# nju-websoft/OpenEA

Hardware: AMD Instinct MI355X
Metric: training triples/sec (k=10 truncated negatives + limited loss + Adagrad) (higher is better)
Workload: dtype f32; 1 GPU; BootEA/AlignE translational step, EN-FR-100K-V1 shape (synthetic), dim=100, GLOBAL batch=20000 positives (weak scaling: 20000 per GPU x 1 GPU), k=10, truncated eps=0.98; the same workload at every N (; global_batch=20000, entities=200000, parallelism=single

## Files before the change

### openea_amd/csrc/triple_step.hip

```cpp
#include <stdlib.h>

#include <algorithm>
#include <vector>

#include "common.h"
#include "step_plan.h"

namespace {

using oea::group_sum;

using oea::flag_t;
using oea::grad_t;

struct StepWs {
    grad_t *ent_grad, *rel_grad;
    grad_t *rel_extra;
    int64_t rel_copy_stride;
    flag_t *ent_touched, *rel_touched;
    grad_t *nrm_grad, *nrm_extra;
    flag_t *nrm_touched;
    double *partials;
    __device__ __forceinline__ grad_t *rel_copy(int64_t c) const {
        return c == 0 ? rel_grad : rel_extra + (c - 1) * rel_copy_stride;
    }
    __device__ __forceinline__ grad_t *nrm_copy(int64_t c) const {
        return c == 0 ? nrm_grad : nrm_extra + (c - 1) * rel_copy_stride;
    }
};
constexpr int kMaxBlocks = 4096;
constexpr int kRelCopies = 16;

static size_t align256(size_t x) { return (x + 255) / 256 * 256; }

static size_t ws_layout(int64_t n_ent, int64_t n_rel, int32_t ld, void *base, StepWs *ws) {
    size_t off = 0;
    char *b = static_cast<char *>(base);
    auto take = [&](size_t bytes) { size_t o = off; off += align256(bytes); return b ? b + o : nullptr; };
    grad_t *eg = (grad_t *)take(sizeof(grad_t) * (size_t)n_ent * ld);
    grad_t *rg = (grad_t *)take(sizeof(grad_t) * (size_t)n_rel * ld);
    grad_t *ng = (grad_t *)take(sizeof(grad_t) * (size_t)n_rel * ld);
    flag_t *et = (flag_t *)take(sizeof(flag_t) * (size_t)n_ent);
    flag_t *rt = (flag_t *)take(sizeof(flag_t) * (size_t)n_rel);
    flag_t *nt = (flag_t *)take(sizeof(flag_t) * (size_t)n_rel);
    grad_t *rx = (grad_t *)take(sizeof(grad_t) * (size_t)n_rel * ld * (kRelCopies - 1));
    grad_t *nx = (grad_t *)take(sizeof(grad_t) * (size_t)n_rel * ld * (kRelCopies - 1));
    double *pp = (double *)take(sizeof(double) * kMaxBlocks);
    if (ws) {
        ws->rel_copy_stride = n_rel * (int64_t)ld; ws->ent_grad = eg; ws->rel_grad = rg; ws->rel_extra = rx;
        ws->ent_touched = et; ws->rel_touched = rt; ws->nrm_grad = ng; ws->nrm_extra = nx; ws->nrm_touched = nt; ws->partials = pp;
    }
    return off;
}

template <int G, int IT>
struct Row {
    float v[IT];
};

template <int G, int IT, bool TIGHT = false>
__device__ __forceinline__ void load_row(const float *__restrict__ base, int ld, int lane, Row<G, IT> &r) {
#pragma unroll
    for (int it = 0; it < IT; ++it) {
        const int c = it * G + lane;
        r.v[it] = ((TIGHT && G == 32 && it < IT - 1) || c < ld) ? base[c] : 0.f;
    }
}
template <int G, int IT>
__device__ __forceinline__ void load_grad_raw(const grad_t *__restrict__ base, int ld, int lane, grad_t (&q)[IT]) {
#pragma unroll
    for (int it = 0; it < IT; ++it) {
        const int c = it * G + lane;
        q[it] = c < ld ? base[c] : (grad_t)0;
    }
}
template <int G, int IT>
__device__ __forceinline__ void load_grad_row(const grad_t *__restrict__ base, int ld, int lane, Row<G, IT> &r) {
#pragma unroll
    for (int it = 0; it < IT; ++it) {
        const int c = it * G + lane;
        r.v[it] = c < ld ? oea::grad_val(base[c]) : 0.f;
    }
}
template <int G, int IT>
__device__ __forceinline__ float sumsq(const Row<G, IT> &r) {
    float s = 0.f;
#pragma unroll
    for (int it = 0; it < IT; ++it) s += r.v[it] * r.v[it];
    return group_sum<G>(s);
}
template <int G, int IT>
__device__ __forceinline__ void normalize(Row<G, IT> &r, int on) {
    if (!on) return;
    const float inv = rsqrtf(fmaxf(sumsq<G, IT>(r), 1e-12f));
#pragma unroll
    for (int it = 0; it < IT; ++it) r.v[it] *= inv;
}
template <int G, int IT>
__device__ __forceinline__ float score(const Row<G, IT> &yh, const Row<G, IT> &yr, const Row<G, IT> &yt, int l1,
                                       Row<G, IT> &delta) {
    float s = 0.f;
#pragma unroll
    for (int it = 0; it < IT; ++it) {
        const float d = yh.v[it] + yr.v[it] - yt.v[it];
        delta.v[it] = d;
        s += l1 ? fabsf(d) : d * d;
    }
    return group_sum<G>(s);
}
__device__ __forceinline__ float sgn(float x) { return x > 0.f ? 1.f : (x < 0.f ? -1.f : 0.f); }

template <int G, int IT>
__device__ __forceinline__ void dscore(const Row<G, IT> &delta, float coef, int l1, Row<G, IT> &g) {
#pragma unroll
    for (int it = 0; it < IT; ++it) g.v[it] = l1 ? coef * sgn(delta.v[it]) : 2.f * coef * delta.v[it];
}
template <int G, int IT, bool SKIPZERO = true>
__device__ __forceinline__ void atomic_row(grad_t *__restrict__ dst, int ld, int lane, const Row<G, IT> &g, float sign) {
#pragma unroll
    for (int it = 0; it < IT; ++it) {
        const int c = it * G + lane;
        const float v = sign * g.v[it];
        if (((G == 32 && it < IT - 1) || c < ld) && (!SKIPZERO || v != 0.f)) oea::grad_add(dst + c, v);
    }
}

__device__ __forceinline__ float softplusf_(float x) { return x > 0.f ? x + log1pf(expf(-x)) : log1pf(expf(x)); }
__device__ __forceinline__ float sigmoidf_(float x) { return 1.f / (1.f + expf(-x)); }

__device__ __forceinline__ void triple_coef_kind(int loss_kind, const oea_step_cfg &cfg, bool is_pos, float s, float &coef,
                                                 float &l) {
    coef = 0.f; l = 0.f;
    switch (loss_kind) {
    case OEA_LOSS_LIMITED:
        if (is_pos) { const float x = s - cfg.pos_margin; if (x > 0.f) { l = x; coef = 1.f; } }
        else { const float x = cfg.neg_margin - s; if (x > 0.f) { l = cfg.balance * x; coef = -cfg.balance; } }
        break;
    case OEA_LOSS_LOGISTIC:
        if (is_pos) { l = softplusf_(s); coef = sigmoidf_(s); }
        else { l = softplusf_(-s); coef = -sigmoidf_(-s); }
        break;
    case OEA_LOSS_POSITIVE:
        l = s; coef = 1.f;
        break;
    case OEA_LOSS_ALIGN:
        l = softplusf_(s); coef = sigmoidf_(s);
        break;
    default: break;
    }
}
__device__ __forceinline__ void triple_coef(const oea_step_cfg &cfg, bool is_pos, float s, float &coef, float &l) {
    triple_coef_kind(cfg.loss_kind, cfg, is_pos, s, coef, l);
}

__device__ __forceinline__ void block_loss_partial(double loss_local, double *partials) {
    __shared__ double sred[4];
    const double w = oea::wave_sum_d(loss_local);
    if ((threadIdx.x & 63) == 0) sred[threadIdx.x >> 6] = w;
    __syncthreads();
    if (threadIdx.x == 0) partials[blockIdx.x] = sred[0] + sred[1] + sred[2] + sred[3];
}

template <int G, int IT>
__global__ __launch_bounds__(256) void triple_generic(
    const float *__restrict__ ent, const float *__restrict__ rel, int ld, const int32_t *__restrict__ pos,
    int64_t n_pos, const int32_t *__restrict__ neg, int64_t n_neg, oea_step_cfg cfg, StepWs ws) {
    const int lane = threadIdx.x % G;
    const int64_t grp = ((int64_t)blockIdx.x * blockDim.x + threadIdx.x) / G;
    const int64_t ngrp = (int64_t)gridDim.x * blockDim.x / G;
    const bool margin = cfg.loss_kind == OEA_LOSS_MARGIN;
    const int64_t items = margin ? n_pos : n_pos + n_neg;
    double loss_local = 0.0;
    for (int64_t item = grp; item < items; item += ngrp) {
        const bool is_pos = margin || item < n_pos;
        const int32_t *tr = is_pos ? pos + 3 * item : neg + 3 * (item - n_pos);
        const int h = tr[0], r = tr[1], t = tr[2];
        Row<G, IT> yh, yr, yt, delta, g;
        load_row<G, IT>(ent + (int64_t)h * ld, ld, lane, yh);
        load_row<G, IT>(rel + (int64_t)r * ld, ld, lane, yr);
        load_row<G, IT>(ent + (int64_t)t * ld, ld, lane, yt);
        normalize<G, IT>(yh, cfg.ent_l2_norm);
        normalize<G, IT>(yr, cfg.rel_l2_norm);
        normalize<G, IT>(yt, cfg.ent_l2_norm);
        const float s = score<G, IT>(yh, yr, yt, cfg.l1, delta);
        float coef, l;
        if (margin) {
            const int32_t *tn = neg + 3 * item;
            const int nh = tn[0], nr = tn[1], nt = tn[2];
            Row<G, IT> zh, zr, zt, dn;
            load_row<G, IT>(ent + (int64_t)nh * ld, ld, lane, zh);
            load_row<G, IT>(rel + (int64_t)nr * ld, ld, lane, zr);
            load_row<G, IT>(ent + (int64_t)nt * ld, ld, lane, zt);
            normalize<G, IT>(zh, cfg.ent_l2_norm);
            normalize<G, IT>(zr, cfg.rel_l2_norm);
            normalize<G, IT>(zt, cfg.ent_l2_norm);
            const float sn = score<G, IT>(zh, zr, zt, cfg.l1, dn);
            const float x = cfg.margin + s - sn;
            if (x <= 0.f) continue;
            if (lane == 0) loss_local += (double)x;
            dscore<G, IT>(dn, -1.f, cfg.l1, g);
            atomic_row<G, IT>(ws.ent_grad + (int64_t)nh * ld, ld, lane, g, 1.f);
            atomic_row<G, IT>(ws.rel_copy(item % kRelCopies) + (int64_t)nr * ld, ld, lane, g, 1.f);
            atomic_row<G, IT>(ws.ent_grad + (int64_t)nt * ld, ld, lane, g, -1.f);
            if (lane == 0) { ws.ent_touched[nh] = 1.f; ws.ent_touched[nt] = 1.f; ws.rel_touched[nr] = 1.f; }
            coef = 1.f;
        } else {
            triple_coef(cfg, is_pos, s, coef, l);
            if (lane == 0) loss_local += (double)l;
            if (coef == 0.f) continue;
        }
        dscore<G, IT>(delta, coef, cfg.l1, g);
        atomic_row<G, IT>(ws.ent_grad + (int64_t)h * ld, ld, lane, g, 1.f);
        atomic_row<G, IT>(ws.rel_copy(item % kRelCopies) + (int64_t)r * ld, ld, lane, g, 1.f);
        atomic_row<G, IT>(ws.ent_grad + (int64_t)t * ld, ld, lane, g, -1.f);
        if (lane == 0) { ws.ent_touched[h] = 1.f; ws.ent_touched[t] = 1.f; ws.rel_touched[r] = 1.f; }
    }
    block_loss_partial(loss_local, ws.partials);
}

template <int G, int IT>
__device__ __forceinline__ double score_independent(const float *__restrict__ ent, const float *__restrict__ rel, int ld,
                                                    int lane, int64_t item, int ch, int cr, int ct, bool is_pos,
                                                    const oea_step_cfg &cfg, const StepWs &ws, int lk, int l1) {
    Row<G, IT> zh, zr, zt, delta, g;
    load_row<G, IT>(ent + (int64_t)ch * ld, ld, lane, zh);
    load_row<G, IT>(rel + (int64_t)cr * ld, ld, lane, zr);
    load_row<G, IT>(ent + (int64_t)ct * ld, ld, lane, zt);
    normalize<G, IT>(zh, cfg.ent_l2_norm);
    normalize<G, IT>(zr, cfg.rel_l2_norm);
    normalize<G, IT>(zt, cfg.ent_l2_norm);
    const float s = score<G, IT>(zh, zr, zt, l1, delta);
    float coef, l;
    triple_coef_kind(lk, cfg, is_pos, s, coef, l);
    if (coef != 0.f) {
        dscore<G, IT>(delta, coef, l1, g);
        atomic_row<G, IT>(ws.ent_grad + (int64_t)ch * ld, ld, lane, g, 1.f);
        atomic_row<G, IT>(ws.rel_copy(item % kRelCopies) + (int64_t)cr * ld, ld, lane, g, 1.f);
        atomic_row<G, IT>(ws.ent_grad + (int64_t)ct * ld, ld, lane, g, -1.f);
        if (lane == 0) { ws.ent_touched[ch] = 1.f; ws.ent_touched[ct] = 1.f; ws.rel_touched[cr] = 1.f; }
    }
    return (double)l;
}

template <int G, int IT, int LOSS, int L1>
__global__ __launch_bounds__(256, (IT <= 4 ? 3 : 2)) void triple_grouped(
    const float *__restrict__ ent, const float *__restrict__ rel, int ld, const int32_t *__restrict__ pos,
    int64_t n_pos, const int32_t *__restrict__ neg, int k, oea_step_cfg cfg, StepWs ws) {
    constexpr int KC = IT <= 4 ? 10 : (IT <= 8 ? 4 : 2);
    static_assert(3 * KC <= G, "ids of a chunk fit one register across the group");
    const int lane = threadIdx.x % G;
    const int64_t grp = ((int64_t)blockIdx.x * blockDim.x + threadIdx.x) / G;
    const int64_t ngrp = (int64_t)gridDim.x * blockDim.x / G;
    const int lk = LOSS >= 0 ? LOSS : cfg.loss_kind;
    const int l1 = L1 >= 0 ? L1 : cfg.l1;
    double loss_local = 0.0;
    for (int64_t p = grp; p < n_pos; p += ngrp) {
        const int32_t *ng = neg + (int64_t)p * k * 3;
        const int pid = lane < 3 ? pos[3 * p + lane] : 0;
        int nid = lane < 3 * min(KC, k) ? ng[lane] : 0;
        const int h = __shfl(pid, 0, G), r = __shfl(pid, 1, G), t = __shfl(pid, 2, G);
        Row<G, IT> yh, yr, yt, delta, g, gh, gr, gt;
        load_row<G, IT, true>(ent + (int64_t)h * ld, ld, lane, yh);
        load_row<G, IT, true>(rel + (int64_t)r * ld, ld, lane, yr);
        load_row<G, IT, true>(ent + (int64_t)t * ld, ld, lane, yt);
        double lsum = 0.0;
        bool any = false;
        for (int base = 0; base < k; base += KC) {
            if (base > 0) nid = lane < 3 * min(KC, k - base) ? ng[3 * base + lane] : 0;
            int ce[KC];
            unsigned tailm = 0, okm = 0, slow = 0;
            Row<G, IT> yc[KC];
#pragma unroll
            for (int j = 0; j < KC; ++j) {
                const int ch = __shfl(nid, 3 * j, G), cr = __shfl(nid, 3 * j + 1, G), ct = __shfl(nid, 3 * j + 2, G);
                const bool valid = base + j < k;
                const bool tl = ch == h;
                const bool ok = valid && cr == r && (tl || ct == t);
                tailm |= tl ? 1u << j : 0u;
                okm |= ok ? 1u << j : 0u;
                slow |= (valid && !ok) ? 1u << j : 0u;
                ce[j] = valid ? (tl ? ct : ch) : h;
                load_row<G, IT, true>(ent + (int64_t)ce[j] * ld, ld, lane, yc[j]);
            }
            if (base == 0) {
                normalize<G, IT>(yh, cfg.ent_l2_norm);
                normalize<G, IT>(yr, cfg.rel_l2_norm);
                normalize<G, IT>(yt, cfg.ent_l2_norm);
                const float s = score<G, IT>(yh, yr, yt, l1, delta);
                float coef, l;
                triple_coef_kind(lk, cfg, true, s, coef, l);
                lsum = (double)l;
                dscore<G, IT>(delta, coef, l1, g);
#pragma unroll
                for (int it = 0; it < IT; ++it) { gh.v[it] = g.v[it]; gr.v[it] = g.v[it]; gt.v[it] = -g.v[it]; }
                any = coef != 0.f;
            }
            if (slow) {
#pragma unroll 1
                for (int j = 0; j < KC; ++j)
                    if ((slow >> j) & 1u)
                        lsum += score_independent<G, IT>(ent, rel, ld, lane, p, __shfl(nid, 3 * j, G), __shfl(nid, 3 * j + 1, G),
                                                         __shfl(nid, 3 * j + 2, G), false, cfg, ws, lk, l1);
            }
            float sc[KC];
#pragma unroll
            for (int j = 0; j < KC; ++j) {
                normalize<G, IT>(yc[j], cfg.ent_l2_norm);
                float s = 0.f;
#pragma unroll
                for (int it = 0; it < IT; ++it) {
                    const bool tl = (tailm >> j) & 1u;
                    const float a = tl ? yh.v[it] : yc[j].v[it], b = tl ? yc[j].v[it] : yt.v[it];
                    const float d = a + yr.v[it] - b;
                    yc[j].v[it] = d;
                    s += l1 ? fabsf(d) : d * d;
                }
                sc[j] = group_sum<G>(s);
            }
#pragma unroll
            for (int j = 0; j < KC; ++j) {
                if (!((okm >> j) & 1u)) continue;
                const bool tl = (tailm >> j) & 1u;
                float coef, l;
                triple_coef_kind(lk, cfg, false, sc[j], coef, l);
                lsum += (double)l;
                if (coef != 0.f) {
                    any = true;
                    dscore<G, IT>(yc[j], coef, l1, g);
                    if (tl) {
#pragma unroll
                        for (int it = 0; it < IT; ++it) { gh.v[it] += g.v[it]; gr.v[it] += g.v[it]; }
                    } else {
#pragma unroll
                        for (int it = 0; it < IT; ++it) { gr.v[it] += g.v[it]; gt.v[it] -= g.v[it]; }
                    }
                    atomic_row<G, IT>(ws.ent_grad + (int64_t)ce[j] * ld, ld, lane, g, tl ? -1.f : 1.f);
                    if (lane == 0) ws.ent_touched[ce[j]] = 1.f;
                }
            }
        }
        if (k <= 0) {
            normalize<G, IT>(yh, cfg.ent_l2_norm);
            normalize<G, IT>(yr, cfg.rel_l2_norm);
            normalize<G, IT>(yt, cfg.ent_l2_norm);
            const float s = score<G, IT>(yh, yr, yt, l1, delta);
            float coef, l;
            triple_coef_kind(lk, cfg, true, s, coef, l);
            lsum = (double)l;
            dscore<G, IT>(delta, coef, l1, g);
#pragma unroll
            for (int it = 0; it < IT; ++it) { gh.v[it] = g.v[it]; gr.v[it] = g.v[it]; gt.v[it] = -g.v[it]; }
            any = coef != 0.f;
        }
        if (any) {
            atomic_row<G, IT>(ws.ent_grad + (int64_t)h * ld, ld, lane, gh, 1.f);
            atomic_row<G, IT>(ws.rel_copy(p % kRelCopies) + (int64_t)r * ld, ld, lane, gr, 1.f);
            atomic_row<G, IT>(ws.ent_grad + (int64_t)t * ld, ld, lane, gt, 1.f);
            if (lane == 0) { ws.ent_touched[h] = 1.f; ws.ent_touched[t] = 1.f; ws.rel_touched[r] = 1.f; }
        }
        if (lane == 0) loss_local += lsum;
    }
    block_loss_partial(loss_local, ws.partials);
}

#ifdef OEA_DET_SCRATCH
constexpr int kGradShift = 3;
#else
constexpr int kGradShift = 2;
#endif
constexpr unsigned kBufFlags = 0x00020000u;
constexpr int kBufRecords = (int)0x80000000u;
constexpr int kBufOob = (int)0xC0000000u;

__device__ __forceinline__ void buf_grad_add(__amdgpu_buffer_rsrc_t rs, float v, int voff, int soff, int imm) {
#ifdef OEA_DET_SCRATCH
    const long long q = oea::to_fixed(v);
    const int vo = voff + imm;
    asm volatile("s_nop 4\n\tbuffer_atomic_add_x2 %0, %1, %2, %3 offen" ::"v"(q), "v"(vo), "s"(rs), "s"(soff) : "memory");
#else
    __builtin_amdgcn_raw_ptr_buffer_atomic_fadd_f32(v, rs, voff + imm, soff, 0);
#endif
}
__device__ __forceinline__ void buf_flag_set(__amdgpu_buffer_rsrc_t rs, int row) {
#ifdef OEA_DET_SCRATCH
    typedef unsigned int u32x2 __attribute__((ext_vector_type(2)));
    const u32x2 one = {1u, 0u};
    __builtin_amdgcn_raw_buffer_store_b64(one, rs, 0, row * 8, 0);
#else
    __builtin_amdgcn_raw_buffer_store_b32(0x3f800000u, rs, 0, row * 4, 0);
#endif
}
template <int IT>
__device__ __forceinline__ void wave_load_row(__amdgpu_buffer_rsrc_t rs, int soff, int v4, int vt, Row<64, IT> &r) {
#pragma unroll
    for (int it = 0; it < IT; ++it)
        r.v[it] = __builtin_bit_cast(float, __builtin_amdgcn_raw_buffer_load_b32(rs, it < IT - 1 ? v4 + it * 256 : vt, soff, 0));
}
template <int IT>
__device__ __forceinline__ void wave_atomic_row(__amdgpu_buffer_rsrc_t rs, int soff, int vg, int vgt, const Row<64, IT> &g, float sign) {
#pragma unroll
    for (int it = 0; it < IT; ++it) {
        if (it < IT - 1) buf_grad_add(rs, sign * g.v[it], vg, soff, it * (64 << kGradShift));
        else buf_grad_add(rs, sign * g.v[it], vgt, soff, 0);
    }
}
template <int IT>
__device__ __forceinline__ void wave_rel_row(const StepWs &ws, int dbg, int64_t p, int r, int row_g, int vg, int vgt, const Row<64, IT> &g) {
    const int copy = (int)(p % kRelCopies);
    grad_t *rgb = copy == 0 ? ws.rel_grad : ws.rel_extra + (copy - 1) * ws.rel_copy_stride;
    const __amdgpu_buffer_rsrc_t rs_rg = __builtin_amdgcn_make_buffer_rsrc(rgb, 0, (dbg & 1) ? 0 : kBufRecords, kBufFlags);
    const __amdgpu_buffer_rsrc_t rs_rt = __builtin_amdgcn_make_buffer_rsrc(ws.rel_touched, 0, (dbg & 4) ? 0 : kBufRecords, kBufFlags);
    wave_atomic_row<IT>(rs_rg, r * row_g, vg, vgt, g, 1.f);
    buf_flag_set(rs_rt, r);
}
__device__ __forceinline__ float uniform_f(float x) {
    return __builtin_bit_cast(float, __builtin_amdgcn_readfirstlane(__builtin_bit_cast(int, x)));
}

__device__ __forceinline__ double uniform_d(double x) {
    const unsigned long long b = __builtin_bit_cast(unsigned long long, x);
    const unsigned lo = (unsigned)__builtin_amdgcn_readfirstlane((int)(unsigned)b), hi = (unsigned)__builtin_amdgcn_readfirstlane((int)(unsigned)(b >> 32));
    return __builtin_bit_cast(double, ((unsigned long long)hi << 32) | lo);
}

template <int IT>
__device__ __forceinline__ void wave_normalize(Row<64, IT> &r) {
    float s = 0.f;
#pragma unroll
    for (int it = 0; it < IT; ++it) s += r.v[it] * r.v[it];
    const float inv = rsqrtf(fmaxf(oea::wave_sum_uniform(s), 1e-12f));
#pragma unroll
    for (int it = 0; it < IT; ++it) r.v[it] *= inv;
}

template <int IT, int L1, int KT, bool PLAN>
__global__ __launch_bounds__(512, (IT <= 2 ? (KT == 10 ? 8 : 7) : 4)) void triple_wave(
    const float *__restrict__ ent, const float *__restrict__ rel, int ld, const int32_t *__restrict__ pos,
    int64_t n_pos, const int32_t *__restrict__ neg, int k, oea_step_cfg cfg, StepWs ws, int dbg, float *__restrict__ contrib,
    const uint32_t *__restrict__ pflags, const uint32_t *__restrict__ order) {
    constexpr int G = 64, KC = 10;
    if (KT > 0) k = KT;
    const int lane = threadIdx.x & 63;
    const int wv = __builtin_amdgcn_readfirstlane((int)(threadIdx.x >> 6));
    const int wpb = blockDim.x >> 6;
    const int64_t nw = (int64_t)gridDim.x * wpb;
    const int row_b = ld * 4, row_g = ld << kGradShift;
    const __amdgpu_buffer_rsrc_t rs_ent = __builtin_amdgcn_make_buffer_rsrc(const_cast<float *>(ent), 0, (dbg & 2) ? 0 : kBufRecords, kBufFlags);
    const __amdgpu_buffer_rsrc_t rs_rel = __builtin_amdgcn_make_buffer_rsrc(const_cast<float *>(rel), 0, (dbg & 2) ? 0 : kBufRecords, kBufFlags);
    const __amdgpu_buffer_rsrc_t rs_eg = __builtin_amdgcn_make_buffer_rsrc(ws.ent_grad, 0, (dbg & 1) ? 0 : kBufRecords, kBufFlags);
    const __amdgpu_buffer_rsrc_t rs_et = __builtin_amdgcn_make_buffer_rsrc(ws.ent_touched, 0, (dbg & 4) ? 0 : kBufRecords, kBufFlags);
    const int v4 = lane * 4, vg = lane << kGradShift;
    const int c_last = (IT - 1) * 64 + lane;
    const int vt = c_last < ld ? c_last * 4 : kBufOob, vgt = c_last < ld ? c_last << kGradShift : kBufOob;
    const float c_neg = L1 ? -cfg.balance : -2.f * cfg.balance;
    double loss_local = 0.0;
    auto score_positive = [&](int64_t p, Row<G, IT> &gacc) -> int {
        const int32_t *pp = pos + 3 * p;
        const int32_t *ng = neg + p * k * 3;
        const int h = pp[0], r = pp[1], t = pp[2];
        Row<G, IT> yh, yr, yt;
        wave_load_row<IT>(rs_ent, h * row_b, v4, vt, yh);
        wave_load_row<IT>(rs_rel, r * row_b, v4, vt, yr);
        wave_load_row<IT>(rs_ent, t * row_b, v4, vt, yt);
        int ids[3 * KC];
        if (KT == KC || k == KC) {
#pragma unroll
            for (int q = 0; q < 3 * KC; ++q) ids[q] = ng[q];
        } else {
#pragma unroll
            for (int q = 0; q < 3 * KC; ++q) ids[q] = q < 3 * k ? ng[q] : 0;
        }
        unsigned bad = 0, xh = 0, xt = 0;
#pragma unroll
        for (int j = 0; j < KC; ++j)
            if (KT == KC || j < k) {
                const unsigned a = (unsigned)(ids[3 * j] ^ h), b = (unsigned)(ids[3 * j + 2] ^ t), c = (unsigned)(ids[3 * j + 1] ^ r);
                bad |= c | min(a, b);
                xh |= a;
                xt |= b;
            }
        if (bad | min(xh, xt)) {
            double ls = score_independent<G, IT>(ent, rel, ld, lane, p, h, r, t, true, cfg, ws, OEA_LOSS_LIMITED, L1);
#pragma unroll 1
            for (int j = 0; j < k; ++j)
                ls += score_independent<G, IT>(ent, rel, ld, lane, p, ng[3 * j], ng[3 * j + 1], ng[3 * j + 2], false, cfg, ws, OEA_LOSS_LIMITED, L1);
            loss_local = uniform_d(loss_local + ls);
            return -1;
        }
        const bool tails = xh == 0;
        int ce[KC];
        Row<G, IT> yc[KC];
#pragma unroll
        for (int j = 0; j < KC; ++j)
            if (KT == KC || j < k) {
                ce[j] = tails ? ids[3 * j + 2] : ids[3 * j];
                wave_load_row<IT>(rs_ent, ce[j] * row_b, v4, vt, yc[j]);
            }
        wave_normalize<IT>(yh);
        wave_normalize<IT>(yr);
        wave_normalize<IT>(yt);
        Row<G, IT> u, gpos;
        int r_sum = -1;
        float sp = 0.f;
#pragma unroll
        for (int it = 0; it < IT; ++it) {
            u.v[it] = yh.v[it] + yr.v[it];
            const float d = u.v[it] - yt.v[it];
            gpos.v[it] = d;
            sp += L1 ? fabsf(d) : d * d;
        }
        const float xp = oea::wave_sum_uniform(sp) - cfg.pos_margin;
        const bool cpos = xp > 0.f;
        float lsum = cpos ? xp : 0.f;
#pragma unroll
        for (int it = 0; it < IT; ++it) {
            gpos.v[it] = cpos ? (L1 ? sgn(gpos.v[it]) : 2.f * gpos.v[it]) : 0.f;
            gacc.v[it] = gpos.v[it];
        }
        float sc[KC];
        if (tails) {
#pragma unroll
            for (int j = 0; j < KC; ++j)
                if (KT == KC || j < k) {
                    wave_normalize<IT>(yc[j]);
                    float s = 0.f;
#pragma unroll
                    for (int it = 0; it < IT; ++it) {
                        const float d = u.v[it] - yc[j].v[it];
                        yc[j].v[it] = d;
                        s += L1 ? fabsf(d) : d * d;
                    }
                    sc[j] = oea::wave_sum_uniform(s);
                }
        } else {
#pragma unroll
            for (int j = 0; j < KC; ++j)
                if (KT == KC || j < k) {
                    wave_normalize<IT>(yc[j]);
                    float s = 0.f;
#pragma unroll
                    for (int it = 0; it < IT; ++it) {
                        const float d = yc[j].v[it] + yr.v[it] - yt.v[it];
                        yc[j].v[it] = d;
                        s += L1 ? fabsf(d) : d * d;
                    }
                    sc[j] = oea::wave_sum_uniform(s);
                }
        }
        bool anyneg = false;
        const float sign_c = tails ? -1.f : 1.f;
#pragma unroll
        for (int j = 0; j < KC; ++j)
            if (KT == KC || j < k) {
                const float xn = cfg.neg_margin - sc[j];
                if (xn > 0.f) {
                    lsum += cfg.balance * xn;
                    anyneg = true;
                    Row<G, IT> g;
#pragma unroll
                    for (int it = 0; it < IT; ++it) {
                        g.v[it] = L1 ? c_neg * sgn(yc[j].v[it]) : c_neg * yc[j].v[it];
                        gacc.v[it] += g.v[it];
                    }
                    wave_atomic_row<IT>(rs_eg, ce[j] * row_g, vg, vgt, g, sign_c);
                    buf_flag_set(rs_et, ce[j]);
                }
            }
        if (PLAN) {
            const __amdgpu_buffer_rsrc_t rs_cb = __builtin_amdgcn_make_buffer_rsrc(contrib, 0, kBufRecords, kBufFlags);
            const int so = (int)p * 2 * row_b;
#pragma unroll
            for (int it = 0; it < IT; ++it) {
                const int vo = it < IT - 1 ? v4 + it * 256 : vt;
                __builtin_amdgcn_raw_buffer_store_b32(__builtin_bit_cast(unsigned, gacc.v[it]), rs_cb, vo, so, 0);
                __builtin_amdgcn_raw_buffer_store_b32(__builtin_bit_cast(unsigned, gpos.v[it]), rs_cb, vo, so + row_b, 0);
            }
        }
        if (cpos | anyneg) {
            if (PLAN && order) r_sum = r;
            else wave_rel_row<IT>(ws, dbg, p, r, row_g, vg, vgt, gacc);
            const unsigned via_atomics = PLAN ? pflags[p] : 3u;
            const bool h_full = tails, t_full = !tails;
            if ((via_atomics & 1u) && (h_full || cpos)) {
                wave_atomic_row<IT>(rs_eg, h * row_g, vg, vgt, h_full ? gacc : gpos, 1.f);
                buf_flag_set(rs_et, h);
            }
            if ((via_atomics & 2u) && (t_full || cpos)) {
                wave_atomic_row<IT>(rs_eg, t * row_g, vg, vgt, t_full ? gacc : gpos, -1.f);
                buf_flag_set(rs_et, t);
            }
        }
        loss_local = uniform_d(loss_local + (double)lsum);
        return r_sum;
    };
    if constexpr (!PLAN) {
        for (int64_t p = (int64_t)blockIdx.x * wpb + wv; p < n_pos; p += nw) {
            Row<G, IT> gacc;
            (void)score_positive(p, gacc);
        }
    } else {
        for (int64_t q0 = (int64_t)blockIdx.x * wpb; q0 < n_pos; q0 += nw) {
            const int64_t q = q0 + wv;
            Row<G, IT> gacc;
            const int r_sum = q < n_pos ? score_positive(order ? (int64_t)order[q] : q, gacc) : -1;
            if (!order) continue;
            __shared__ float s_row[8][IT][64];
            __shared__ int s_rel[8];
            int lb = v4;
            asm volatile("" : "+v"(lb));
            const auto at = [lb](auto *base) { return (decltype(base))((char *)base + lb); };
            if (lb == 0) s_rel[wv] = r_sum;
            if (r_sum >= 0) {
#pragma unroll
                for (int it = 0; it < IT; ++it) *at(&s_row[wv][it][0]) = gacc.v[it];
            }
            __syncthreads();
            if (r_sum >= 0) {
                const int held = lb < wpb * 4 ? *at(&s_rel[0]) : -1;
                bool first = true;
#pragma unroll
                for (int w = 0; w < 8; ++w) first = first && !(w < wv && __builtin_amdgcn_readlane(held, w) == r_sum);
                if (first) {
#pragma unroll
                    for (int w = 1; w < 8; ++w)
                        if (w > wv && __builtin_amdgcn_readlane(held, w) == r_sum) {
#pragma unroll
                            for (int it = 0; it < IT; ++it) gacc.v[it] += *at(&s_row[w][it][0]);
                        }
                    wave_rel_row<IT>(ws, dbg, order[q], r_sum, row_g, vg, vgt, gacc);
                }
            }
            if (q0 + nw < n_pos) __syncthreads();
        }
    }
    __shared__ double sred[8];
    int lz = v4;
    if constexpr (PLAN) asm volatile("" : "+v"(lz));
    if (lz == 0) sred[wv] = loss_local;
    __syncthreads();
    if (wv == 0 && lz == 0) {
        double s = 0.0;
        for (int w = 0; w < wpb; ++w) s += sred[w];
        ws.partials[blockIdx.x] = s;
    }
}

template <int G, int IT>
__device__ __forceinline__ float dot(const Row<G, IT> &a, const Row<G, IT> &b) {
    float s = 0.f;
#pragma unroll
    for (int it = 0; it < IT; ++it) s += a.v[it] * b.v[it];
    return group_sum<G>(s);
}
template <int G, int IT>
__device__ __forceinline__ void load_normal(const float *__restrict__ nrm, int r, int ld, int lane, Row<G, IT> &yn) {
    load_row<G, IT>(nrm + (int64_t)r * ld, ld, lane, yn);
    normalize<G, IT>(yn, 1);
    normalize<G, IT>(yn, 1);
}
template <int G, int IT>
__device__ double transh_independent(const float *__restrict__ ent, const float *__restrict__ rel, int ld, int lane,
                                     int64_t item, int h, int r, int t, bool is_pos, const oea_step_cfg &cfg,
                                     const StepWs &ws) {
    Row<G, IT> yh, yr, yt, yn, delta, g;
    load_row<G, IT>(ent + (int64_t)h * ld, ld, lane, yh);
    load_row<G, IT>(rel + (int64_t)r * ld, ld, lane, yr);
    load_row<G, IT>(ent + (int64_t)t * ld, ld, lane, yt);
    load_normal<G, IT>(cfg.normal, r, ld, lane, yn);
    normalize<G, IT>(yh, cfg.ent_l2_norm);
    normalize<G, IT>(yr, cfg.rel_l2_norm);
    normalize<G, IT>(yt, cfg.ent_l2_norm);
    const float ah = dot<G, IT>(yh, yn), at = dot<G, IT>(yt, yn);
    float s = 0.f;
#pragma unroll
    for (int it = 0; it < IT; ++it) {
        const float d = (yh.v[it] - ah * yn.v[it]) + yr.v[it] - (yt.v[it] - at * yn.v[it]);
        delta.v[it] = d;
        s += cfg.l1 ? fabsf(d) : d * d;
    }
    s = group_sum<G>(s);
    float coef, l;
    triple_coef(cfg, is_pos, s, coef, l);
    if (coef != 0.f) {
        dscore<G, IT>(delta, coef, cfg.l1, g);
        const float gdn = dot<G, IT>(g, yn);
        Row<G, IT> pg, gn;
#pragma unroll
        for (int it = 0; it < IT; ++it) {
            pg.v[it] = g.v[it] - gdn * yn.v[it];
            gn.v[it] = (at - ah) * g.v[it] + gdn * (yt.v[it] - yh.v[it]);
        }
        atomic_row<G, IT>(ws.ent_grad + (int64_t)h * ld, ld, lane, pg, 1.f);
        atomic_row<G, IT>(ws.ent_grad + (int64_t)t * ld, ld, lane, pg, -1.f);
        atomic_row<G, IT>(ws.rel_copy(item % kRelCopies) + (int64_t)r * ld, ld, lane, g, 1.f);
        atomic_row<G, IT>(ws.nrm_copy(item % kRelCopies) + (int64_t)r * ld, ld, lane, gn, 1.f);
        if (lane == 0) { ws.ent_touched[h] = 1.f; ws.ent_touched[t] = 1.f; ws.rel_touched[r] = 1.f; ws.nrm_touched[r] = 1.f; }
    }
    return (double)l;
}

template <int G, int IT>
__global__ __launch_bounds__(256) void triple_transh_grouped(
    const float *__restrict__ ent, const float *__restrict__ rel, int ld, const int32_t *__restrict__ pos,
    int64_t n_pos, const int32_t *__restrict__ neg, int k, oea_step_cfg cfg, StepWs ws) {
    const int lane = threadIdx.x % G;
    const int64_t grp = ((int64_t)blockIdx.x * blockDim.x + threadIdx.x) / G;
    const int64_t ngrp = (int64_t)gridDim.x * blockDim.x / G;
    double loss_local = 0.0;
    for (int64_t p = grp; p < n_pos; p += ngrp) {
        const int h = pos[3 * p], r = pos[3 * p + 1], t = pos[3 * p + 2];
        const int32_t *ng = neg + (int64_t)p * k * 3;
        Row<G, IT> yh, yr, yt, yn, ph, pt, g, gh, gr, gt, gn;
        load_row<G, IT>(ent + (int64_t)h * ld, ld, lane, yh);
        load_row<G, IT>(rel + (int64_t)r * ld, ld, lane, yr);
        load_row<G, IT>(ent + (int64_t)t * ld, ld, lane, yt);
        load_normal<G, IT>(cfg.normal, r, ld, lane, yn);
        normalize<G, IT>(yh, cfg.ent_l2_norm);
        normalize<G, IT>(yr, cfg.rel_l2_norm);
        normalize<G, IT>(yt, cfg.ent_l2_norm);
        const float ah = dot<G, IT>(yh, yn), at = dot<G, IT>(yt, yn);
        float s = 0.f;
#pragma unroll
        for (int it = 0; it < IT; ++it) {
            ph.v[it] = yh.v[it] - ah * yn.v[it];
            pt.v[it] = yt.v[it] - at * yn.v[it];
            const float d = ph.v[it] + yr.v[it] - pt.v[it];
            g.v[it] = d;
            s += cfg.l1 ? fabsf(d) : d * d;
        }
        s = group_sum<G>(s);
        float coef, l;
        triple_coef(cfg, true, s, coef, l);
        double lsum = (double)l;
        bool any = coef != 0.f;
        {
            Row<G, IT> d0 = g;
            dscore<G, IT>(d0, coef, cfg.l1, g);
            const float gdn = dot<G, IT>(g, yn);
#pragma unroll
            for (int it = 0; it < IT; ++it) {
                const float pg = g.v[it] - gdn * yn.v[it];
                gh.v[it] = pg; gt.v[it] = -pg; gr.v[it] = g.v[it];
                gn.v[it] = (at - ah) * g.v[it] + gdn * (yt.v[it] - yh.v[it]);
            }
        }
        for (int j0 = 0; j0 < k; j0 += 2) {
            int ch[2], cr[2], ct[2];
            Row<G, IT> yc[2];
#pragma unroll
            for (int u = 0; u < 2; ++u) {
                const int j = j0 + u < k ? j0 + u : j0;
                ch[u] = ng[3 * j]; cr[u] = ng[3 * j + 1]; ct[u] = ng[3 * j + 2];
                load_row<G, IT>(ent + (int64_t)((ch[u] == h) ? ct[u] : ch[u]) * ld, ld, lane, yc[u]);
            }
#pragma unroll
            for (int u = 0; u < 2; ++u) {
                if (j0 + u >= k) continue;
                const bool tail = ch[u] == h;
                if (!(cr[u] == r && (tail || ct[u] == t))) {
                    lsum += transh_independent<G, IT>(ent, rel, ld, lane, p, ch[u], cr[u], ct[u], false, cfg, ws);
                    continue;
                }
                const int ce = tail ? ct[u] : ch[u];
                normalize<G, IT>(yc[u], cfg.ent_l2_norm);
                const float ac = dot<G, IT>(yc[u], yn);
                Row<G, IT> delta;
                s = 0.f;
#pragma unroll
                for (int it = 0; it < IT; ++it) {
                    const float pc = yc[u].v[it] - ac * yn.v[it];
                    const float d = tail ? ph.v[it] + yr.v[it] - pc : pc + yr.v[it] - pt.v[it];
                    delta.v[it] = d;
                    s += cfg.l1 ? fabsf(d) : d * d;
                }
                s = group_sum<G>(s);
                triple_coef(cfg, false, s, coef, l);
                lsum += (double)l;
                if (coef == 0.f) continue;
                any = true;
                dscore<G, IT>(delta, coef, cfg.l1, g);
                const float gdn = dot<G, IT>(g, yn);
                Row<G, IT> pg;
#pragma unroll
                for (int it = 0; it < IT; ++it) {
                    pg.v[it] = g.v[it] - gdn * yn.v[it];
                    gr.v[it] += g.v[it];
                    if (tail) {
                        gh.v[it] += pg.v[it];
                        gn.v[it] += (ac - ah) * g.v[it] + gdn * (yc[u].v[it] - yh.v[it]);
                    } else {
                        gt.v[it] -= pg.v[it];
                        gn.v[it] += (at - ac) * g.v[it] + gdn * (yt.v[it] - yc[u].v[it]);
                    }
                }
                atomic_row<G, IT>(ws.ent_grad + (int64_t)ce * ld, ld, lane, pg, tail ? -1.f : 1.f);
                if (lane == 0) ws.ent_touched[ce] = 1.f;
            }
        }
        if (any) {
            atomic_row<G, IT>(ws.ent_grad + (int64_t)h * ld, ld, lane, gh, 1.f);
            atomic_row<G, IT>(ws.ent_grad + (int64_t)t * ld, ld, lane, gt, 1.f);
            atomic_row<G, IT>(ws.rel_copy(p % kRelCopies) + (int64_t)r * ld, ld, lane, gr, 1.f);
            atomic_row<G, IT>(ws.nrm_copy(p % kRelCopies) + (int64_t)r * ld, ld, lane, gn, 1.f);
            if (lane == 0) { ws.ent_touched[h] = 1.f; ws.ent_touched[t] = 1.f; ws.rel_touched[r] = 1.f; ws.nrm_touched[r] = 1.f; }
        }
        if (lane == 0) loss_local += lsum;
    }
    block_loss_partial(loss_local, ws.partials);
}

template <int G, int IT>
__device__ float transd_triple(const float *__restrict__ ent, const float *__restrict__ rel, int ld, int lane,
                               int64_t item, int h, int r, int t, bool is_pos, const oea_step_cfg &cfg,
                               const StepWs &ws, int mode, float coef, float &l) {
    const int64_t eb = cfg.ent_transfer_base, rb = cfg.rel_transfer_base;
    Row<G, IT> yh, yt, yr, hp, tp, rp, H, T, g;
    load_row<G, IT>(ent + (int64_t)h * ld, ld, lane, yh);
    load_row<G, IT>(ent + (int64_t)t * ld, ld, lane, yt);
    load_row<G, IT>(rel + (int64_t)r * ld, ld, lane, yr);
    load_row<G, IT>(ent + (eb + h) * ld, ld, lane, hp);
    load_row<G, IT>(ent + (eb + t) * ld, ld, lane, tp);
    load_row<G, IT>(rel + (rb + r) * ld, ld, lane, rp);
    normalize<G, IT>(yh, cfg.ent_l2_norm);
    normalize<G, IT>(yt, cfg.ent_l2_norm);
    normalize<G, IT>(yr, cfg.rel_l2_norm);
    normalize<G, IT>(hp, cfg.ent_l2_norm);
    normalize<G, IT>(tp, cfg.ent_l2_norm);
    normalize<G, IT>(rp, cfg.rel_l2_norm);
    const float ah = dot<G, IT>(yh, hp), at = dot<G, IT>(yt, tp);
#pragma unroll
    for (int it = 0; it < IT; ++it) {
        H.v[it] = yh.v[it] + ah * rp.v[it];
        T.v[it] = yt.v[it] + at * rp.v[it];
    }
    const float ssh = sumsq<G, IT>(H), sst = sumsq<G, IT>(T);
    const float ih = rsqrtf(fmaxf(ssh, 1e-12f)), itl = rsqrtf(fmaxf(sst, 1e-12f));
    float s = 0.f;
#pragma unroll
    for (int it = 0; it < IT; ++it) {
        H.v[it] *= ih;
        T.v[it] *= itl;
        const float d = H.v[it] + yr.v[it] - T.v[it];
        g.v[it] = d;
        s += cfg.l1 ? fabsf(d) : d * d;
    }
    s = group_sum<G>(s);
    l = 0.f;
    if (mode == 0) return s;
    if (mode == 2) triple_coef(cfg, is_pos, s, coef, l);
    if (coef == 0.f) return s;
    {
        Row<G, IT> d0 = g;
        dscore<G, IT>(d0, coef, cfg.l1, g);
    }
    const float ch = ssh > 1e-12f ? dot<G, IT>(g, H) : 0.f, ct = sst > 1e-12f ? dot<G, IT>(g, T) : 0.f;
    Row<G, IT> qh, qt;
#pragma unroll
    for (int it = 0; it < IT; ++it) {
        qh.v[it] = (g.v[it] - ch * H.v[it]) * ih;
        qt.v[it] = (ct * T.v[it] - g.v[it]) * itl;
    }
    const float bh = dot<G, IT>(qh, rp), bt = dot<G, IT>(qt, rp);
    Row<G, IT> o;
#pragma unroll
    for (int it = 0; it < IT; ++it) o.v[it] = qh.v[it] + bh * hp.v[it];
    atomic_row<G, IT>(ws.ent_grad + (int64_t)h * ld, ld, lane, o, 1.f);
#pragma unroll
    for (int it = 0; it < IT; ++it) o.v[it] = bh * yh.v[it];
    atomic_row<G, IT>(ws.ent_grad + (eb + h) * ld, ld, lane, o, 1.f);
#pragma unroll
    for (int it = 0; it < IT; ++it) o.v[it] = qt.v[it] + bt * tp.v[it];
    atomic_row<G, IT>(ws.ent_grad + (int64_t)t * ld, ld, lane, o, 1.f);
#pragma unroll
    for (int it = 0; it < IT; ++it) o.v[it] = bt * yt.v[it];
    atomic_row<G, IT>(ws.ent_grad + (eb + t) * ld, ld, lane, o, 1.f);
#pragma unroll
    for (int it = 0; it < IT; ++it) o.v[it] = ah * qh.v[it] + at * qt.v[it];
    atomic_row<G, IT>(ws.rel_copy(item % kRelCopies) + (rb + r) * ld, ld, lane, o, 1.f);
    atomic_row<G, IT>(ws.rel_copy(item % kRelCopies) + (int64_t)r * ld, ld, lane, g, 1.f);
    if (lane == 0) {
        ws.ent_touched[h] = 1.f; ws.ent_touched[t] = 1.f; ws.ent_touched[eb + h] = 1.f; ws.ent_touched[eb + t] = 1.f;
        ws.rel_touched[r] = 1.f; ws.rel_touched[rb + r] = 1.f;
    }
    return s;
}

template <int G, int IT>
__device__ float transh_triple(const float *__restrict__ ent, const float *__restrict__ rel, int ld, int lane,
                               int64_t item, int h, int r, int t, bool is_pos, const oea_step_cfg &cfg,
                               const StepWs &ws, int mode, float coef, float &l) {
    Row<G, IT> yh, yr, yt, yn, g;
    load_row<G, IT>(ent + (int64_t)h * ld, ld, lane, yh);
    load_row<G, IT>(rel + (int64_t)r * ld, ld, lane, yr);
    load_row<G, IT>(ent + (int64_t)t * ld, ld, lane, yt);
    load_normal<G, IT>(cfg.normal, r, ld, lane, yn);
    normalize<G, IT>(yh, cfg.ent_l2_norm);
// ... 1781 lines not shown
```

Measured before the change: 283.3 million triples/s.

## Add fused mixed-side negative path and specialize one-sided path at compile time

Triples whose negatives corrupt a mix of heads and tails were previously sent to a slow independent per-negative scoring fallback. They now go through a register-resident path that picks head or tail per negative from a bitmask and issues atomics directly to the entity rows. The existing one-sided path is wrapped in a lambda templated on the side, so the tails/heads branch is resolved at compile time. This trades extra code size and register pressure, and more atomics per negative in the mixed path (no gacc merging for h/t, no plan contributions), for avoiding the fallback.

```diff
diff --git a/openea_amd/csrc/triple_step.hip b/openea_amd/csrc/triple_step.hip
--- a/openea_amd/csrc/triple_step.hip
+++ b/openea_amd/csrc/triple_step.hip
@@ -1,6 +1,7 @@
 #include <stdlib.h>
 
 #include <algorithm>
+#include <type_traits>
 #include <vector>
 
 #include "common.h"
@@ -479,7 +480,7 @@
                 xh |= a;
                 xt |= b;
             }
-        if (bad | min(xh, xt)) {
+        if (bad) {
             double ls = score_independent<G, IT>(ent, rel, ld, lane, p, h, r, t, true, cfg, ws, OEA_LOSS_LIMITED, L1);
 #pragma unroll 1
             for (int j = 0; j < k; ++j)
@@ -487,111 +488,203 @@
             loss_local = uniform_d(loss_local + ls);
             return -1;
         }
-        const bool tails = xh == 0;
-        int ce[KC];
-        Row<G, IT> yc[KC];
-#pragma unroll
-        for (int j = 0; j < KC; ++j)
-            if (KT == KC || j < k) {
-                ce[j] = tails ? ids[3 * j + 2] : ids[3 * j];
-                wave_load_row<IT>(rs_ent, ce[j] * row_b, v4, vt, yc[j]);
-            }
-        wave_normalize<IT>(yh);
-        wave_normalize<IT>(yr);
-        wave_normalize<IT>(yt);
-        Row<G, IT> u, gpos;
-        int r_sum = -1;
-        float sp = 0.f;
-#pragma unroll
-        for (int it = 0; it < IT; ++it) {
-            u.v[it] = yh.v[it] + yr.v[it];
-            const float d = u.v[it] - yt.v[it];
-            gpos.v[it] = d;
-            sp += L1 ? fabsf(d) : d * d;
-        }
-        const float xp = oea::wave_sum_uniform(sp) - cfg.pos_margin;
-        const bool cpos = xp > 0.f;
-        float lsum = cpos ? xp : 0.f;
-#pragma unroll
-        for (int it = 0; it < IT; ++it) {
-            gpos.v[it] = cpos ? (L1 ? sgn(gpos.v[it]) : 2.f * gpos.v[it]) : 0.f;
-            gacc.v[it] = gpos.v[it];
-        }
-        float sc[KC];
-        if (tails) {
+        if (min(xh, xt)) {
+            unsigned tmask = 0;
+            int ce[KC];
+            Row<G, IT> yc[KC];
 #pragma unroll
             for (int j = 0; j < KC; ++j)
                 if (KT == KC || j < k) {
+                    const int nh = ids[3 * j], nt = ids[3 * j + 2];
+                    const bool tl = nh == h;
+                    tmask |= tl ? 1u << j : 0u;
+                    ce[j] = tl ? nt : nh;
+                    wave_load_row<IT>(rs_ent, ce[j] * row_b, v4, vt, yc[j]);
+                }
+            asm volatile("" : "+s"(tmask));
+#pragma unroll
+            for (int it = 0; it < IT; ++it)
+                asm volatile("" : "+v"(yh.v[it]), "+v"(yr.v[it]), "+v"(yt.v[it]));
+            wave_normalize<IT>(yh);
+            wave_normalize<IT>(yr);
+            wave_normalize<IT>(yt);
+            Row<G, IT> u, gpos;
+            float sp = 0.f;
+#pragma unroll
+            for (int it = 0; it < IT; ++it) {
+                u.v[it] = yh.v[it] + yr.v[it];
+                const float d = u.v[it] - yt.v[it];
+                gpos.v[it] = d;
+                sp += L1 ? fabsf(d) : d * d;
+            }
+            const float xp = oea::wave_sum_uniform(sp) - cfg.pos_margin;
+            const bool cpos = xp > 0.f;
+            float lsum = cpos ? xp : 0.f;
+#pragma unroll
+            for (int it = 0; it < IT; ++it) {
+                gpos.v[it] = cpos ? (L1 ? sgn(gpos.v[it]) : 2.f * gpos.v[it]) : 0.f;
+                gacc.v[it] = gpos.v[it];
+            }
+            bool anyneg = false;
+#pragma unroll
+            for (int j = 0; j < KC; ++j)
+                if (KT == KC || j < k) {
+                    const bool tl = (tmask >> j) & 1u;
                     wave_normalize<IT>(yc[j]);
                     float s = 0.f;
-#pragma unroll
-                    for (int it = 0; it < IT; ++it) {
-                        const float d = u.v[it] - yc[j].v[it];
-                        yc[j].v[it] = d;
-                        s += L1 ? fabsf(d) : d * d;
+                    if (tl) {
+#pragma unroll
+                        for (int it = 0; it < IT; ++it) {
+                            const float d = u.v[it] - yc[j].v[it];
+                            yc[j].v[it] = d;
+                            s += L1 ? fabsf(d) : d * d;
+                        }
+                    } else {
+#pragma unroll
+                        for (int it = 0; it < IT; ++it) {
+                            const float d = yc[j].v[it] + yr.v[it] - yt.v[it];
+                            yc[j].v[it] = d;
+                            s += L1 ? fabsf(d) : d * d;
+                        }
                     }
-                    sc[j] = oea::wave_sum_uniform(s);
+                    const float xn = cfg.neg_margin - oea::wave_sum_uniform(s);
+                    if (xn > 0.f) {
+                        lsum += cfg.balance * xn;
+                        anyneg = true;
+                        Row<G, IT> g;
+#pragma unroll
+                        for (int it = 0; it < IT; ++it) {
+                            g.v[it] = L1 ? c_neg * sgn(yc[j].v[it]) : c_neg * yc[j].v[it];
+                            gacc.v[it] += g.v[it];
+                        }
+                        const int pe = tl ? h : t;
+                        const float sign_c = tl ? -1.f : 1.f;
+                        wave_atomic_row<IT>(rs_eg, ce[j] * row_g, vg, vgt, g, sign_c);
+                        buf_flag_set(rs_et, ce[j]);
+                        wave_atomic_row<IT>(rs_eg, pe * row_g, vg, vgt, g, -sign_c);
+                        buf_flag_set(rs_et, pe);
+                    }
                 }
-        } else {
+            if (cpos) {
+                wave_atomic_row<IT>(rs_eg, h * row_g, vg, vgt, gpos, 1.f);
+                buf_flag_set(rs_et, h);
+                wave_atomic_row<IT>(rs_eg, t * row_g, vg, vgt, gpos, -1.f);
+                buf_flag_set(rs_et, t);
+            }
+            loss_local = uniform_d(loss_local + (double)lsum);
+            if (!(cpos | anyneg)) return -1;
+            if (PLAN && order) return r;
+            wave_rel_row<IT>(ws, dbg, p, r, row_g, vg, vgt, gacc);
+            return -1;
+        }
+        auto one_sided = [&](auto side) -> int {
+            constexpr bool tails = decltype(side)::value;
+            int ce[KC];
+            Row<G, IT> yc[KC];
 #pragma unroll
             for (int j = 0; j < KC; ++j)
                 if (KT == KC || j < k) {
-                    wave_normalize<IT>(yc[j]);
-                    float s = 0.f;
-#pragma unroll
-                    for (int it = 0; it < IT; ++it) {
-                        const float d = yc[j].v[it] + yr.v[it] - yt.v[it];
-                        yc[j].v[it] = d;
-                        s += L1 ? fabsf(d) : d * d;
+                    ce[j] = tails ? ids[3 * j + 2] : ids[3 * j];
+                    wave_load_row<IT>(rs_ent, ce[j] * row_b, v4, vt, yc[j]);
+                }
+            wave_normalize<IT>(yh);
+            wave_normalize<IT>(yr);
+            wave_normalize<IT>(yt);
+            Row<G, IT> u, gpos;
+            int r_sum = -1;
+            float sp = 0.f;
+#pragma unroll
+            for (int it = 0; it < IT; ++it) {
+                u.v[it] = yh.v[it] + yr.v[it];
+                const float d = u.v[it] - yt.v[it];
+                gpos.v[it] = d;
+                sp += L1 ? fabsf(d) : d * d;
+            }
+            const float xp = oea::wave_sum_uniform(sp) - cfg.pos_margin;
+            const bool cpos = xp > 0.f;
+            float lsum = cpos ? xp : 0.f;
+#pragma unroll
+            for (int it = 0; it < IT; ++it) {
+                gpos.v[it] = cpos ? (L1 ? sgn(gpos.v[it]) : 2.f * gpos.v[it]) : 0.f;
+                gacc.v[it] = gpos.v[it];
+            }
+            float sc[KC];
+            if (tails) {
+#pragma unroll
+                for (int j = 0; j < KC; ++j)
+                    if (KT == KC || j < k) {
+                        wave_normalize<IT>(yc[j]);
+                        float s = 0.f;
+#pragma unroll
+                        for (int it = 0; it < IT; ++it) {
+                            const float d = u.v[it] - yc[j].v[it];
+                            yc[j].v[it] = d;
+                            s += L1 ? fabsf(d) : d * d;
+                        }
+                        sc[j] = oea::wave_sum_uniform(s);
                     }
-                    sc[j] = oea::wave_sum_uniform(s);
+            } else {
+#pragma unroll
+                for (int j = 0; j < KC; ++j)
+                    if (KT == KC || j < k) {
+                        wave_normalize<IT>(yc[j]);
+                        float s = 0.f;
+#pragma unroll
+                        for (int it = 0; it < IT; ++it) {
+                            const float d = yc[j].v[it] + yr.v[it] - yt.v[it];
+                            yc[j].v[it] = d;
+                            s += L1 ? fabsf(d) : d * d;
+                        }
+                        sc[j] = oea::wave_sum_uniform(s);
+                    }
+            }
+            bool anyneg = false;
+            const float sign_c = tails ? -1.f : 1.f;
+#pragma unroll
+            for (int j = 0; j < KC; ++j)
+                if (KT == KC || j < k) {
+                    const float xn = cfg.neg_margin - sc[j];
+                    if (xn > 0.f) {
+                        lsum += cfg.balance * xn;
+                        anyneg = true;
+                        Row<G, IT> g;
+#pragma unroll
+                        for (int it = 0; it < IT; ++it) {
+                            g.v[it] = L1 ? c_neg * sgn(yc[j].v[it]) : c_neg * yc[j].v[it];
+                            gacc.v[it] += g.v[it];
+                        }
+                        wave_atomic_row<IT>(rs_eg, ce[j] * row_g, vg, vgt, g, sign_c);
+                        buf_flag_set(rs_et, ce[j]);
+                    }
                 }
-        }
-        bool anyneg = false;
-        const float sign_c = tails ? -1.f : 1.f;
-#pragma unroll
-        for (int j = 0; j < KC; ++j)
-            if (KT == KC || j < k) {
-                const float xn = cfg.neg_margin - sc[j];
-                if (xn > 0.f) {
-                    lsum += cfg.balance * xn;
-                    anyneg = true;
-                    Row<G, IT> g;
-#pragma unroll
-                    for (int it = 0; it < IT; ++it) {
-                        g.v[it] = L1 ? c_neg * sgn(yc[j].v[it]) : c_neg * yc[j].v[it];
-                        gacc.v[it] += g.v[it];
-                    }
-                    wave_atomic_row<IT>(rs_eg, ce[j] * row_g, vg, vgt, g, sign_c);
-                    buf_flag_set(rs_et, ce[j]);
+            if (PLAN) {
+                const __amdgpu_buffer_rsrc_t rs_cb = __builtin_amdgcn_make_buffer_rsrc(contrib, 0, kBufRecords, kBufFlags);
+                const int so = (int)p * 2 * row_b;
+#pragma unroll
+                for (int it = 0; it < IT; ++it) {
+                    const int vo = it < IT - 1 ? v4 + it * 256 : vt;
+                    __builtin_amdgcn_raw_buffer_store_b32(__builtin_bit_cast(unsigned, gacc.v[it]), rs_cb, vo, so, 0);
+                    __builtin_amdgcn_raw_buffer_store_b32(__builtin_bit_cast(unsigned, gpos.v[it]), rs_cb, vo, so + row_b, 0);
                 }
             }
-        if (PLAN) {
-            const __amdgpu_buffer_rsrc_t rs_cb = __builtin_amdgcn_make_buffer_rsrc(contrib, 0, kBufRecords, kBufFlags);
-            const int so = (int)p * 2 * row_b;
-#pragma unroll
-            for (int it = 0; it < IT; ++it) {
-                const int vo = it < IT - 1 ? v4 + it * 256 : vt;
-                __builtin_amdgcn_raw_buffer_store_b32(__builtin_bit_cast(unsigned, gacc.v[it]), rs_cb, vo, so, 0);
-                __builtin_amdgcn_raw_buffer_store_b32(__builtin_bit_cast(unsigned, gpos.v[it]), rs_cb, vo, so + row_b, 0);
-            }
-        }
-        if (cpos | anyneg) {
-            if (PLAN && order) r_sum = r;
-            else wave_rel_row<IT>(ws, dbg, p, r, row_g, vg, vgt, gacc);
-            const unsigned via_atomics = PLAN ? pflags[p] : 3u;
-            const bool h_full = tails, t_full = !tails;
-            if ((via_atomics & 1u) && (h_full || cpos)) {
-                wave_atomic_row<IT>(rs_eg, h * row_g, vg, vgt, h_full ? gacc : gpos, 1.f);
-                buf_flag_set(rs_et, h);
-            }
-            if ((via_atomics & 2u) && (t_full || cpos)) {
-                wave_atomic_row<IT>(rs_eg, t * row_g, vg, vgt, t_full ? gacc : gpos, -1.f);
-                buf_flag_set(rs_et, t);
-            }
-        }
-        loss_local = uniform_d(loss_local + (double)lsum);
-        return r_sum;
+            if (cpos | anyneg) {
+                if (PLAN && order) r_sum = r;
+                else wave_rel_row<IT>(ws, dbg, p, r, row_g, vg, vgt, gacc);
+                const unsigned via_atomics = PLAN ? pflags[p] : 3u;
+                const bool h_full = tails, t_full = !tails;
+                if ((via_atomics & 1u) && (h_full || cpos)) {
+                    wave_atomic_row<IT>(rs_eg, h * row_g, vg, vgt, h_full ? gacc : gpos, 1.f);
+                    buf_flag_set(rs_et, h);
+                }
+                if ((via_atomics & 2u) && (t_full || cpos)) {
+                    wave_atomic_row<IT>(rs_eg, t * row_g, vg, vgt, t_full ? gacc : gpos, -1.f);
+                    buf_flag_set(rs_et, t);
+                }
+            }
+            loss_local = uniform_d(loss_local + (double)lsum);
+            return r_sum;
+        };
+        return xh == 0 ? one_sided(std::true_type{}) : one_sided(std::false_type{});
     };
     if constexpr (!PLAN) {
         for (int64_t p = (int64_t)blockIdx.x * wpb + wv; p < n_pos; p += nw) {
```

Result: faster. 292.3 million triples/s (median of 6 runs) (+3.2%).
